# crowsonkb/k-diffusion

Hardware: NVIDIA H100
Metric: images/sec (256x256, Heun 50-step) (higher is better)
Workload: dtype bf16

## Files before the change

k-diffusion_b200/csrc/tc_attention.cu:

```cuda
#include "tc_common.cuh"
#include "tc_kernels.cuh"

namespace kdb {
namespace {

constexpr int ROWS = 128, DH = 64;
constexpr int TILE_BYTES = ROWS * DH * 2;
constexpr float LOG2E = 1.4426950408889634f;
constexpr int S_LD = ROWS + 4;

enum { MODE_WINDOW = 0, MODE_GLOBAL = 1, MODE_NA = 2 };

constexpr int NA_QH = 8, NA_QW = 16;
constexpr int NA_KH = 14, NA_KW = 22;
constexpr int NA_BLK_ROWS = 5;
constexpr int NA_BLK_KEYS = NA_BLK_ROWS * NA_KW;

struct AttnParams {
  bf16* out;
  const float* bound;
  int B, h, w, nh, shift, nblk;
};

struct Bars {
  uint64_t q, kv, kv_free;
};

template <int MODE, bool BOUNDED>
__global__ void __launch_bounds__(160, 1) attn_tc_kernel(const __grid_constant__ CUtensorMap tmap, const __grid_constant__ CUtensorMap tmap_kv,
                                                         const AttnParams p) {
  extern __shared__ uint8_t smem_raw[];
  uint8_t* base = reinterpret_cast<uint8_t*>((reinterpret_cast<uintptr_t>(smem_raw) + 1023) & ~(uintptr_t)1023);
  uint8_t* sQ = base;
  uint8_t* sK = base + TILE_BYTES;
  uint8_t* sV = base + 2 * TILE_BYTES;
  uint8_t* sP = (MODE == MODE_WINDOW) ? sQ : base + 3 * TILE_BYTES;
  float* sS = reinterpret_cast<float*>(base + (MODE == MODE_WINDOW ? 3 : 5) * TILE_BYTES);
  Bars* bars = reinterpret_cast<Bars*>(sS + ROWS * S_LD);

  const int warp = threadIdx.x >> 5, lane = threadIdx.x & 31;
  const int nh = p.nh;
  int b = blockIdx.z, head0, wi = 0, wj = 0, mtile = 0;
  if constexpr (MODE == MODE_WINDOW) {
    const int nww = p.w / 8;
    wi = blockIdx.x / nww;
    wj = blockIdx.x - wi * nww;
    head0 = blockIdx.y * 2;
  } else {
    mtile = blockIdx.x;
    head0 = blockIdx.y;
  }
  int qi0 = 0, qj0 = 0, r0 = 0, c0 = 0;
  if constexpr (MODE == MODE_NA) {
    const int nbw = p.w / NA_QW;
    qi0 = (blockIdx.x / nbw) * NA_QH;
    qj0 = (blockIdx.x % nbw) * NA_QW;
    r0 = min(max(qi0 - 3, 0), p.h - NA_KH);
    c0 = min(max(qj0 - 3, 0), p.w - NA_KW);
  }
  const int nblk = (MODE == MODE_WINDOW) ? 1 : p.nblk;
  constexpr bool bounded = BOUNDED;
  const bool two_pass = nblk > 1 && !bounded;
  const int n_iter = two_pass ? 2 * nblk : nblk;

  if (threadIdx.x == 0) {
    tc::tma_prefetch_desc(&tmap);
    tc::mbar_init(&bars->q, 1);
    tc::mbar_init(&bars->kv, 1);
    tc::mbar_init(&bars->kv_free, 4);
    tc::fence_barrier_init();
  }
  if constexpr (MODE == MODE_NA) {
    for (int i = threadIdx.x; i < (ROWS - NA_BLK_KEYS) * 8; i += blockDim.x)
      *reinterpret_cast<uint4*>(sV + NA_BLK_KEYS * 128 + i * 16) = make_uint4(0u, 0u, 0u, 0u);
    tc::fence_proxy_async();
  }
  __syncthreads();
  tc::pdl_wait();
  tc::pdl_launch_dependents();

  if (warp == 4) {
    if (tc::elect_one()) {
      auto load_window_tile = [&](uint8_t* dst, int t, uint64_t* bar) {
        if (p.shift == 0) {
#pragma unroll
          for (int hd = 0; hd < 2; ++hd) tc::tma_load_4d(dst + hd * 64 * 128, &tmap, bar, (t * nh + head0 + hd) * DH, wj * 8, wi * 8, b);
          return;
        }
#pragma unroll
        for (int hd = 0; hd < 2; ++hd)
#pragma unroll
          for (int quad = 0; quad < 4; ++quad) {
            const int r0 = (wi * 8 + (quad >> 1) * 4 - p.shift + p.h) % p.h;
            const int c0 = (wj * 8 + (quad & 1) * 4 - p.shift + p.w) % p.w;
            tc::tma_load_4d(dst + (hd * 64 + quad * 16) * 128, &tmap, bar, (t * nh + head0 + hd) * DH, c0, r0, b);
          }
      };
      tc::mbar_arrive_expect_tx(&bars->q, TILE_BYTES);
      if constexpr (MODE == MODE_WINDOW)
        load_window_tile(sQ, 0, &bars->q);
      else if constexpr (MODE == MODE_NA)
        tc::tma_load_4d(sQ, &tmap, &bars->q, head0 * DH, qj0, qi0, b);
      else
        tc::tma_load_3d(sQ, &tmap, &bars->q, head0 * DH, mtile * ROWS, b);
      for (int it = 0; it < n_iter; ++it) {
        const int j = it % nblk;
        const bool with_v = !two_pass || it >= nblk;
        if (it > 0) tc::mbar_wait(&bars->kv_free, (uint32_t)(it - 1) & 1u);
        constexpr uint32_t KV_BYTES = (MODE == MODE_NA) ? NA_BLK_KEYS * 128 : TILE_BYTES;
        tc::mbar_arrive_expect_tx(&bars->kv, with_v ? 2 * KV_BYTES : KV_BYTES);
        if constexpr (MODE == MODE_WINDOW) {
          load_window_tile(sK, 1, &bars->kv);
          load_window_tile(sV, 2, &bars->kv);
        } else if constexpr (MODE == MODE_NA) {
          tc::tma_load_4d(sK, &tmap_kv, &bars->kv, (nh + head0) * DH, c0, r0 + j * NA_BLK_ROWS, b);
          if (with_v) tc::tma_load_4d(sV, &tmap_kv, &bars->kv, (2 * nh + head0) * DH, c0, r0 + j * NA_BLK_ROWS, b);
        } else {
          tc::tma_load_3d(sK, &tmap, &bars->kv, (nh + head0) * DH, j * ROWS, b);
          if (with_v) tc::tma_load_3d(sV, &tmap, &bars->kv, (2 * nh + head0) * DH, j * ROWS, b);
        }
      }
    }
    return;
  }

  const int row = warp * 32 + lane;
  float m = -INFINITY, l = 0.f;
  const int hd = row >> 6, quad = (row & 63) >> 4;
  const bool seam_r = MODE == MODE_WINDOW && p.shift > 0 && wi == 0;
  const bool seam_c = MODE == MODE_WINDOW && p.shift > 0 && wj == 0;
  const int na_qi = qi0 + (row >> 4), na_qj = qj0 + (row & 15);
  const int na_rs = min(max(na_qi - 3, 0), p.h - 7), na_cs = min(max(na_qj - 3, 0), p.w - 7);
  auto key_ok = [&](int j, int t) -> bool {
    if constexpr (MODE != MODE_NA) return true;
    const int dr = (t * 745) >> 14;
    const int kr = r0 + j * NA_BLK_ROWS + dr, kc = c0 + (t - dr * NA_KW);
    return t < NA_BLK_KEYS && (unsigned)(kr - na_rs) < 7u && (unsigned)(kc - na_cs) < 7u;
  };
  const uint32_t q_addr = tc::smem_u32(sQ), k_addr = tc::smem_u32(sK), p_addr = tc::smem_u32(sP);
  const uint64_t vdesc = tc::smem_desc_mn_sw128(tc::smem_u32(sV), 1024, 1024);
  float o0[32], o1[32];
#pragma unroll
  for (int i = 0; i < 32; ++i) o0[i] = o1[i] = 0.f;
  tc::mbar_wait(&bars->q, 0);
  for (int it = 0; it < n_iter; ++it) {
    const int j = it % nblk;
    const int pass = (two_pass && it < nblk) ? 0 : 1;
    tc::mbar_wait(&bars->kv, (uint32_t)it & 1u);
#pragma unroll 1
    for (int h = 0; h < 2; ++h) {
      float s[64];
#pragma unroll
      for (int i = 0; i < 64; ++i) s[i] = 0.f;
      const uint64_t qd = tc::smem_desc_k_sw128(q_addr + (uint32_t)h * 8192u), kd = tc::smem_desc_k_sw128(k_addr);
      tc::wg_fence_acc(s);
      tc::wg_fence();
#pragma unroll
      for (int k = 0; k < DH / 16; ++k) tc::wgmma_128(s, qd + 2ull * k, kd + 2ull * k, 1u);
      tc::wg_commit();
      tc::wg_wait<0>();
      tc::wg_fence_acc(s);
      tc::acc_store(sS, S_LD, 64 * h, s);
    }
    tc::named_barrier_sync(1, 128);
    if (pass == 0) {
#pragma unroll 1
      for (int c = 0; c < 4; ++c) {
        float v[32];
        tc::acc_ld32(sS, S_LD, row, c * 32, v);
#pragma unroll
        for (int i = 0; i < 32; ++i) m = fmaxf(m, key_ok(j, c * 32 + i) ? v[i] : -INFINITY);
      }
    } else if constexpr (MODE != MODE_WINDOW) {
      if constexpr (bounded) m = __ldg(p.bound + head0);
      if (!two_pass && !bounded) {
        float mm = -INFINITY;
#pragma unroll 1
        for (int c2 = 0; c2 < 4; ++c2) {
          float u[32];
          tc::acc_ld32(sS, S_LD, row, c2 * 32, u);
#pragma unroll
          for (int i = 0; i < 32; ++i) mm = fmaxf(mm, u[i]);
        }
        m = mm;
      }
      const float mb = m * LOG2E;
#pragma unroll 1
      for (int c = 0; c < 4; ++c) {
        float v[32];
        tc::acc_ld32(sS, S_LD, row, c * 32, v);
        uint32_t pk[16];
#pragma unroll
        for (int i = 0; i < 16; ++i) {
          const float p0 = key_ok(j, c * 32 + 2 * i) ? exp2f(fmaf(v[2 * i], LOG2E, -mb)) : 0.f;
          const float p1 = key_ok(j, c * 32 + 2 * i + 1) ? exp2f(fmaf(v[2 * i + 1], LOG2E, -mb)) : 0.f;
          pk[i] = tc::pack_bf16x2(p0, p1);
          float q0, q1;
          tc::unpack_bf16x2(pk[i], q0, q1);
          l += q0 + q1;
        }
        uint8_t* pt = sP + (c >> 1) * TILE_BYTES;
#pragma unroll
        for (int jj = 0; jj < 4; ++jj)
          *reinterpret_cast<uint4*>(pt + tc::sw128_offset(row, (c & 1) * 4 + jj)) = make_uint4(pk[jj * 4], pk[jj * 4 + 1], pk[jj * 4 + 2], pk[jj * 4 + 3]);
      }
    } else {
      float v[64];
      {
        float t0[32], t1[32];
        tc::acc_ld32(sS, S_LD, row, hd * 64, t0);
        tc::acc_ld32(sS, S_LD, row, hd * 64 + 32, t1);
#pragma unroll
        for (int i = 0; i < 32; ++i) { v[i] = t0[i]; v[32 + i] = t1[i]; }
      }
      if constexpr (!bounded) {
#pragma unroll
        for (int i = 0; i < 64; ++i) {
          const int kq = i >> 4;
          const bool ok = (!seam_r || ((kq >> 1) == (quad >> 1))) && (!seam_c || ((kq & 1) == (quad & 1)));
          v[i] = ok ? v[i] : -INFINITY;
          m = fmaxf(m, v[i]);
        }
      } else {
        m = __ldg(p.bound + head0 + hd);
      }
      const float mb = m * LOG2E;
      uint8_t* own = sP + hd * TILE_BYTES;
      uint8_t* other = sP + (1 - hd) * TILE_BYTES;
#pragma unroll
      for (int jj = 0; jj < 8; ++jj) {
        uint32_t pk[4];
        bool ok = true;
        if constexpr (bounded) {
          const int kq = jj >> 1;
          ok = (!seam_r || ((kq >> 1) == (quad >> 1))) && (!seam_c || ((kq & 1) == (quad & 1)));
        }
#pragma unroll
        for (int t = 0; t < 4; ++t) {
          float p0 = exp2f(fmaf(v[jj * 8 + 2 * t], LOG2E, -mb)), p1 = exp2f(fmaf(v[jj * 8 + 2 * t + 1], LOG2E, -mb));
          if constexpr (bounded) {
            p0 = ok ? p0 : 0.f;
            p1 = ok ? p1 : 0.f;
          }
          pk[t] = tc::pack_bf16x2(p0, p1);
          float q0, q1;
          tc::unpack_bf16x2(pk[t], q0, q1);
          l += q0 + q1;
        }
        *reinterpret_cast<uint4*>(own + tc::sw128_offset(row, jj)) = make_uint4(pk[0], pk[1], pk[2], pk[3]);
        *reinterpret_cast<uint4*>(other + tc::sw128_offset(row, jj)) = make_uint4(0u, 0u, 0u, 0u);
      }
    }
    if (pass == 1) {
      tc::fence_proxy_async();
      tc::named_barrier_sync(1, 128);
      tc::wg_fence_acc(o0);
      tc::wg_fence_acc(o1);
      tc::wg_fence();
#pragma unroll
      for (int k = 0; k < ROWS / 16; ++k) {
        const uint32_t pa = p_addr + (uint32_t)((k >> 2) * TILE_BYTES);
        const uint64_t bd = vdesc + (uint64_t)(k * ((16 * 128) >> 4));
        tc::wgmma_64<1>(o0, tc::smem_desc_k_sw128(pa) + 2ull * (k & 3), bd, 1u);
        tc::wgmma_64<1>(o1, tc::smem_desc_k_sw128(pa + 8192u) + 2ull * (k & 3), bd, 1u);
      }
      tc::wg_commit();
      tc::wg_wait<0>();
      tc::wg_fence_acc(o0);
      tc::wg_fence_acc(o1);
    }
    tc::named_barrier_sync(1, 128);
    if (lane == 0 && it + 1 < n_iter) tc::mbar_arrive(&bars->kv_free);
  }
  tc::acc_store(sS, S_LD, 0, o0);
  tc::acc_store(sS, S_LD, 64, o1);
  tc::named_barrier_sync(1, 128);
  const float inv = 1.f / l;
  int64_t token;
  int head;
  if constexpr (MODE == MODE_WINDOW) {
    int oi, oj;
    if (p.shift == 0) {
      oi = wi * 8 + ((row & 63) >> 3);
      oj = wj * 8 + (row & 7);
    } else {
      const int lr = (row & 15) >> 2, lc = row & 3;
      oi = (wi * 8 + (quad >> 1) * 4 + lr - p.shift + p.h) % p.h;
      oj = (wj * 8 + (quad & 1) * 4 + lc - p.shift + p.w) % p.w;
    }
    token = (int64_t)oi * p.w + oj;
    head = head0 + hd;
  } else if constexpr (MODE == MODE_NA) {
    token = (int64_t)na_qi * p.w + na_qj;
    head = head0;
  } else {
    token = (int64_t)mtile * ROWS + row;
    head = head0;
  }
  uint4* dst = reinterpret_cast<uint4*>(p.out + (((int64_t)b * p.h * p.w + token) * nh + head) * DH);
#pragma unroll 1
  for (int c = 0; c < 2; ++c) {
// ... 106 lines not shown
```

k-diffusion_b200/csrc/tc_attn_block.cuh:

```cuda
#pragma once

constexpr int AB_C = 128;
constexpr int AB_XBUF = 2;
constexpr int AB_X_BYTES = 2 * A_STAGE_BYTES;
constexpr int AB_WQKV_KB = 3 * AB_C * 128;
constexpr int AB_WO_BYTES = 2 * A_STAGE_BYTES;
constexpr int AB_KV_BYTES = 64 * 128;
constexpr int AB_THREADS = 256 + 32;

struct AttnBlockBars {
  uint64_t w_full, x_full[AB_XBUF], x_empty[AB_XBUF];
};
constexpr size_t AB_SMEM = (size_t)AB_XBUF * AB_X_BYTES + 2 * AB_WQKV_KB + AB_WO_BYTES + 4 * AB_KV_BYTES + sizeof(AttnBlockBars) + 1024;

struct AttnBlockParams {
  const float* ss_in;
  float* ss_out;
  const float4* rope;
  const float* qk_scale;
  int h, w, shift, nwin;
};

__device__ __forceinline__ void ab_window(const AttnBlockParams& p, int win, int& b, int& wi, int& wj) {
  const int nww = p.w >> 3, per_img = (p.h >> 3) * nww;
  b = win / per_img;
  const int rem = win - b * per_img;
  wi = rem / nww;
  wj = rem - wi * nww;
}
__device__ __forceinline__ void ab_quad(const AttnBlockParams& p, int wi, int wj, int q, int& r, int& c) {
  r = (wi * 8 + (q >> 1) * 4 - p.shift + p.h) % p.h;
  c = (wj * 8 + (q & 1) * 4 - p.shift + p.w) % p.w;
}

__global__ void __launch_bounds__(AB_THREADS, 1) gemm_wg_attn_block_kernel(const __grid_constant__ CUtensorMap tmx,
                                                                          const __grid_constant__ CUtensorMap tmwq,
                                                                          const __grid_constant__ CUtensorMap tmwo, const AttnBlockParams p) {
  extern __shared__ uint8_t smem_raw[];
  uint8_t* base = reinterpret_cast<uint8_t*>((reinterpret_cast<uintptr_t>(smem_raw) + 1023) & ~(uintptr_t)1023);
  uint8_t* sX = base;
  uint8_t* sWQ = sX + AB_XBUF * AB_X_BYTES;
  uint8_t* sWO = sWQ + 2 * AB_WQKV_KB;
  uint8_t* sKV = sWO + AB_WO_BYTES;
  AttnBlockBars* bars = reinterpret_cast<AttnBlockBars*>(sKV + 4 * AB_KV_BYTES);
  const int pwarp = threadIdx.x >> 5, lane = threadIdx.x & 31;
  const int n_tiles = (p.nwin + 1) >> 1;
  const int n_local = (int)blockIdx.x < n_tiles ? (n_tiles - 1 - (int)blockIdx.x) / (int)gridDim.x + 1 : 0;

  if (threadIdx.x == 0) {
    tc::tma_prefetch_desc(&tmx);
    tc::tma_prefetch_desc(&tmwq);
    tc::tma_prefetch_desc(&tmwo);
    tc::mbar_init(&bars->w_full, 1);
    for (int i = 0; i < AB_XBUF; ++i) {
      tc::mbar_init(&bars->x_full[i], 1);
      tc::mbar_init(&bars->x_empty[i], 2);
    }
    tc::fence_barrier_init();
  }
  __syncthreads();
  tc::pdl_wait();
  tc::pdl_launch_dependents();

  if (pwarp == 8) {
    if (tc::elect_one()) {
      tc::mbar_arrive_expect_tx(&bars->w_full, 2 * AB_WQKV_KB + AB_WO_BYTES);
#pragma unroll
      for (int kb = 0; kb < 2; ++kb) {
        tc::tma_load_2d(sWQ + kb * AB_WQKV_KB, &tmwq, &bars->w_full, kb * BK, 0);
        tc::tma_load_2d(sWQ + kb * AB_WQKV_KB + 192 * 128, &tmwq, &bars->w_full, kb * BK, 192);
        tc::tma_load_2d(sWO + kb * A_STAGE_BYTES, &tmwo, &bars->w_full, kb * BK, 0);
      }
      for (int i = 0; i < n_local; ++i) {
        const int buf = i & 1;
        const int win0 = 2 * ((int)blockIdx.x + i * (int)gridDim.x);
        const int nw = p.nwin - win0 < 2 ? 1 : 2;
        tc::mbar_wait_nocall(&bars->x_empty[buf], (uint32_t)(((i >> 1) & 1) ^ 1));
        tc::mbar_arrive_expect_tx(&bars->x_full[buf], (uint32_t)nw * 2u * AB_KV_BYTES);
        for (int s = 0; s < nw; ++s) {
          int b, wi, wj;
          ab_window(p, win0 + s, b, wi, wj);
#pragma unroll
          for (int q = 0; q < 4; ++q) {
            int r, c;
            ab_quad(p, wi, wj, q, r, c);
#pragma unroll
            for (int kb = 0; kb < 2; ++kb)
              tc::tma_load_4d(sX + (size_t)buf * AB_X_BYTES + kb * A_STAGE_BYTES + s * AB_KV_BYTES + q * 2048, &tmx, &bars->x_full[buf], kb * BK, c, r, b);
          }
        }
      }
    }
    return;
  }

  const int wg = pwarp >> 2, t = threadIdx.x & 127;
  const int rw = 16 * (t >> 5) + (lane >> 2);
  const int r0 = 64 * wg + rw;
  const int cq = 2 * (lane & 3);
  const int quad = rw >> 4, lr = (rw & 15) >> 2, lc = rw & 3;
  uint8_t* sK = sKV + wg * 2 * AB_KV_BYTES;
  uint8_t* sV = sK + AB_KV_BYTES;
  const uint32_t wq_base = tc::smem_u32(sWQ), wo_base = tc::smem_u32(sWO);
  const uint64_t kdesc = tc::smem_desc_k_sw128(tc::smem_u32(sK));
  const uint64_t vdesc = tc::smem_desc_mn_sw128(tc::smem_u32(sV), 1024, 1024);
  const float sqs[2] = {sqrtf(__ldg(p.qk_scale)), sqrtf(__ldg(p.qk_scale + 1))};
  const int T = p.h * p.w;
  constexpr float LOG2E = 1.4426950408889634f;

  auto store_tile = [&](uint8_t* dst, const float (&a)[32]) {
#pragma unroll
    for (int j = 0; j < 8; ++j) {
      *reinterpret_cast<uint32_t*>(dst + tc::sw128_offset(rw, j) + cq * 2) = tc::pack_bf16x2(a[4 * j], a[4 * j + 1]);
      *reinterpret_cast<uint32_t*>(dst + tc::sw128_offset(rw + 8, j) + cq * 2) = tc::pack_bf16x2(a[4 * j + 2], a[4 * j + 3]);
    }
  };
  auto qk_norm_rope = [&](float (&a)[32], int hd, int tok0, int tok1) {
    float4 cs[2][2];
#pragma unroll
    for (int jj = 0; jj < 2; ++jj) {
      const float4* tb = p.rope + (int64_t)(hd * 8 + 4 * jj + (lane & 3)) * T;
      cs[0][jj] = __ldg(tb + tok0);
      cs[1][jj] = __ldg(tb + tok1);
    }
    const float sq = sqs[hd];
    float s0 = 0.f, s1 = 0.f;
#pragma unroll
    for (int j = 0; j < 8; ++j) {
      s0 = fmaf(a[4 * j], a[4 * j], fmaf(a[4 * j + 1], a[4 * j + 1], s0));
      s1 = fmaf(a[4 * j + 2], a[4 * j + 2], fmaf(a[4 * j + 3], a[4 * j + 3], s1));
    }
    s0 += __shfl_xor_sync(0xffffffffu, s0, 1);
    s0 += __shfl_xor_sync(0xffffffffu, s0, 2);
    s1 += __shfl_xor_sync(0xffffffffu, s1, 1);
    s1 += __shfl_xor_sync(0xffffffffu, s1, 2);
    const float sc[2] = {sq * rsqrtf(s0 + 1e-6f), sq * rsqrtf(s1 + 1e-6f)};
#pragma unroll
    for (int jj = 0; jj < 2; ++jj)
#pragma unroll
      for (int rr = 0; rr < 2; ++rr) {
        const int i1 = 4 * jj + 2 * rr, i2 = 4 * (jj + 2) + 2 * rr;
        const float4 c = cs[rr][jj];
        const float x1a = a[i1], x1b = a[i1 + 1], x2a = a[i2], x2b = a[i2 + 1];
        a[i1] = fmaf(x2a, -c.z, x1a * c.x) * sc[rr];
        a[i1 + 1] = fmaf(x2b, -c.w, x1b * c.y) * sc[rr];
        a[i2] = fmaf(x1a, c.z, x2a * c.x) * sc[rr];
        a[i2 + 1] = fmaf(x1b, c.w, x2b * c.y) * sc[rr];
      }
#pragma unroll
    for (int j = 4; j < 8; ++j) {
      a[4 * j] *= sc[0];
      a[4 * j + 1] *= sc[0];
      a[4 * j + 2] *= sc[1];
      a[4 * j + 3] *= sc[1];
    }
  };
  auto to_afrag = [](const float (&a)[32], uint32_t (&f)[16]) {
#pragma unroll
    for (int i = 0; i < 16; ++i) f[i] = tc::pack_bf16x2(a[2 * i], a[2 * i + 1]);
  };

  tc::mbar_wait_nocall(&bars->w_full, 0);
  for (int i = 0; i < n_local; ++i) {
    const int buf = i & 1;
    const int win = 2 * ((int)blockIdx.x + i * (int)gridDim.x) + wg;
    if (win >= p.nwin) continue;
    int b, wi, wj, qr, qc;
    ab_window(p, win, b, wi, wj);
    ab_quad(p, wi, wj, quad, qr, qc);
    const int tok0 = (qr + lr) * p.w + qc + lc, tok1 = tok0 + 2 * p.w;
    const int64_t m0 = (int64_t)b * T + tok0, m1 = (int64_t)b * T + tok1;
    const float rstd0 = rsqrtf(__ldg(p.ss_in + m0 * SS_PARTS) / (float)AB_C + 1e-6f);
    const float rstd1 = rsqrtf(__ldg(p.ss_in + m1 * SS_PARTS) / (float)AB_C + 1e-6f);
    const bool seam_r = p.shift > 0 && wi == 0, seam_c = p.shift > 0 && wj == 0;
    tc::mbar_wait_nocall(&bars->x_full[buf], (uint32_t)((i >> 1) & 1));
    const uint32_t xa = tc::smem_u32(sX + (size_t)buf * AB_X_BYTES) + (uint32_t)wg * AB_KV_BYTES;
    uint32_t of[2][16];
#pragma unroll 1
    for (int hd = 0; hd < 2; ++hd) {
      float va[32], ka[32], qa[32];
#pragma unroll
      for (int j = 0; j < 32; ++j) va[j] = ka[j] = qa[j] = 0.f;
      tc::wg_fence_acc(va);
      tc::wg_fence_acc(ka);
      tc::wg_fence();
      auto project = [&](float (&d)[32], int third) {
#pragma unroll
        for (int kb = 0; kb < 2; ++kb) {
          const uint64_t ad = tc::smem_desc_k_sw128(xa + (uint32_t)(kb * A_STAGE_BYTES));
          const uint64_t bd = tc::smem_desc_k_sw128(wq_base + (uint32_t)(kb * AB_WQKV_KB + (third * AB_C + 64 * hd) * 128));
#pragma unroll
          for (int k = 0; k < 4; ++k) tc::wgmma_64<0>(d, ad + 2ull * k, bd + 2ull * k, 1u);
        }
        tc::wg_commit();
      };
      project(va, 2);
      project(ka, 1);
      if (hd == 1) tc::named_barrier_sync(1 + wg, 128);
      tc::wg_wait<1>();
      tc::wg_fence_acc(va);
#pragma unroll
      for (int j = 0; j < 8; ++j) {
        va[4 * j] *= rstd0;
        va[4 * j + 1] *= rstd0;
        va[4 * j + 2] *= rstd1;
        va[4 * j + 3] *= rstd1;
      }
      store_tile(sV, va);
      tc::wg_fence_acc(qa);
      tc::wg_fence();
      project(qa, 0);
      tc::wg_wait<1>();
      tc::wg_fence_acc(ka);
      qk_norm_rope(ka, hd, tok0, tok1);
      store_tile(sK, ka);
      tc::wg_wait<0>();
      tc::wg_fence_acc(qa);
      qk_norm_rope(qa, hd, tok0, tok1);
      uint32_t qf[16];
      to_afrag(qa, qf);
      tc::fence_proxy_async();
      tc::named_barrier_sync(1 + wg, 128);
      float s[32];
#pragma unroll
      for (int j = 0; j < 32; ++j) s[j] = 0.f;
      tc::wg_fence_acc(s);
      tc::wg_fence_acc(qf);
      tc::wg_fence();
#pragma unroll
      for (int kk = 0; kk < 4; ++kk) {
        const uint32_t a[4] = {qf[4 * kk], qf[4 * kk + 1], qf[4 * kk + 2], qf[4 * kk + 3]};
        tc::wgmma_64_rs<0>(s, a, kdesc + 2ull * kk, 1u);
      }
      tc::wg_commit();
      tc::wg_wait<0>();
      tc::wg_fence_acc(s);
      float mx0 = -INFINITY, mx1 = -INFINITY;
#pragma unroll
      for (int j = 0; j < 8; ++j) {
        const int kq = j >> 1;
        const bool ok = (!seam_r || ((kq >> 1) == (quad >> 1))) && (!seam_c || ((kq & 1) == (quad & 1)));
        if (!ok) s[4 * j] = s[4 * j + 1] = s[4 * j + 2] = s[4 * j + 3] = -INFINITY;
        mx0 = fmaxf(mx0, fmaxf(s[4 * j], s[4 * j + 1]));
        mx1 = fmaxf(mx1, fmaxf(s[4 * j + 2], s[4 * j + 3]));
      }
      mx0 = fmaxf(mx0, __shfl_xor_sync(0xffffffffu, mx0, 1));
      mx0 = fmaxf(mx0, __shfl_xor_sync(0xffffffffu, mx0, 2));
      mx1 = fmaxf(mx1, __shfl_xor_sync(0xffffffffu, mx1, 1));
      mx1 = fmaxf(mx1, __shfl_xor_sync(0xffffffffu, mx1, 2));
      const float mb0 = mx0 * LOG2E, mb1 = mx1 * LOG2E;
      uint32_t pf[16];
      float l0 = 0.f, l1 = 0.f;
#pragma unroll
      for (int i2 = 0; i2 < 16; ++i2) {
        const float mb = (i2 & 1) ? mb1 : mb0;
        pf[i2] = tc::pack_bf16x2(exp2f(fmaf(s[2 * i2], LOG2E, -mb)), exp2f(fmaf(s[2 * i2 + 1], LOG2E, -mb)));
        float e0, e1;
        tc::unpack_bf16x2(pf[i2], e0, e1);
        if (i2 & 1) l1 += e0 + e1;
        else l0 += e0 + e1;
      }
      l0 += __shfl_xor_sync(0xffffffffu, l0, 1);
      l0 += __shfl_xor_sync(0xffffffffu, l0, 2);
      l1 += __shfl_xor_sync(0xffffffffu, l1, 1);
      l1 += __shfl_xor_sync(0xffffffffu, l1, 2);
      float o[32];
#pragma unroll
      for (int j = 0; j < 32; ++j) o[j] = 0.f;
      tc::wg_fence_acc(o);
      tc::wg_fence_acc(pf);
      tc::wg_fence();
#pragma unroll
      for (int kk = 0; kk < 4; ++kk) {
        const uint32_t a[4] = {pf[4 * kk], pf[4 * kk + 1], pf[4 * kk + 2], pf[4 * kk + 3]};
        tc::wgmma_64_rs<1>(o, a, vdesc + (uint64_t)(kk * ((16 * 128) >> 4)), 1u);
      }
      tc::wg_commit();
      tc::wg_wait<0>();
      tc::wg_fence_acc(o);
      const float inv0 = __frcp_rn(l0), inv1 = __frcp_rn(l1);
#pragma unroll
      for (int j = 0; j < 8; ++j) {
        o[4 * j] *= inv0;
        o[4 * j + 1] *= inv0;
        o[4 * j + 2] *= inv1;
        o[4 * j + 3] *= inv1;
      }
      uint32_t oh[16];
      to_afrag(o, oh);
#pragma unroll
      for (int j = 0; j < 16; ++j) {
        of[0][j] = hd == 0 ? oh[j] : of[0][j];
        of[1][j] = hd == 0 ? of[1][j] : oh[j];
      }
    }
    float acc[64];
#pragma unroll
    for (int j = 0; j < 64; ++j) acc[j] = 0.f;
    tc::wg_fence_acc(acc);
    tc::wg_fence_acc(of[0]);
    tc::wg_fence_acc(of[1]);
    tc::wg_fence();
#pragma unroll
    for (int hd = 0; hd < 2; ++hd) {
      const uint64_t od = tc::smem_desc_k_sw128(wo_base + (uint32_t)(hd * A_STAGE_BYTES));
#pragma unroll
      for (int kk = 0; kk < 4; ++kk) {
        const uint32_t a[4] = {of[hd][4 * kk], of[hd][4 * kk + 1], of[hd][4 * kk + 2], of[hd][4 * kk + 3]};
        tc::wgmma_128_rs(acc, a, od + 2ull * kk, 1u);
      }
    }
    tc::wg_commit();
    tc::wg_wait<0>();
    tc::wg_fence_acc(acc);
    uint8_t* xt = sX + (size_t)buf * AB_X_BYTES;
    float ss0 = 0.f, ss1 = 0.f;
#pragma unroll
    for (int j = 0; j < 16; ++j) {
      uint8_t* sub = xt + (j >> 3) * A_STAGE_BYTES;
      uint32_t* p0 = reinterpret_cast<uint32_t*>(sub + tc::sw128_offset(r0, j & 7) + cq * 2);
      uint32_t* p1 = reinterpret_cast<uint32_t*>(sub + tc::sw128_offset(r0 + 8, j & 7) + cq * 2);
      const uint32_t x0 = *p0, x1 = *p1;
      const float a0 = acc[4 * j] + __uint_as_float(x0 << 16), a1 = acc[4 * j + 1] + __uint_as_float(x0 & 0xffff0000u);
      const float b0 = acc[4 * j + 2] + __uint_as_float(x1 << 16), b1 = acc[4 * j + 3] + __uint_as_float(x1 & 0xffff0000u);
      ss0 = fmaf(a0, a0, fmaf(a1, a1, ss0));
      ss1 = fmaf(b0, b0, fmaf(b1, b1, ss1));
      *p0 = tc::pack_bf16x2(a0, a1);
      *p1 = tc::pack_bf16x2(b0, b1);
    }
    ss0 += __shfl_xor_sync(0xffffffffu, ss0, 1);
    ss0 += __shfl_xor_sync(0xffffffffu, ss0, 2);
    ss1 += __shfl_xor_sync(0xffffffffu, ss1, 1);
    ss1 += __shfl_xor_sync(0xffffffffu, ss1, 2);
    if ((lane & 3) == 0) {
      p.ss_out[m0 * SS_PARTS] = ss0;
      p.ss_out[m1 * SS_PARTS] = ss1;
    }
    tc::fence_proxy_async();
    tc::named_barrier_sync(1 + wg, 128);
    if (t == 0) {
#pragma unroll
      for (int q = 0; q < 4; ++q) {
        int r, c;
        ab_quad(p, wi, wj, q, r, c);
#pragma unroll
        for (int kb = 0; kb < 2; ++kb) tc::tma_store_4d(&tmx, xt + kb * A_STAGE_BYTES + wg * AB_KV_BYTES + q * 2048, kb * BK, c, r, b);
      }
      tc::tma_store_commit();
      tc::tma_store_wait_read();
      tc::mbar_arrive(&bars->x_empty[buf]);
    }
  }
}

inline bool attn_block_supported(int h, int w, int C, int nh, int e, int attn_type, int attn_param, int shift) {
  return C == AB_C && nh == 2 && e == 64 && attn_type == KDB_ATTN_SHIFTED_WINDOW && attn_param == 8 && (shift == 0 || shift == 4) && h > 0 &&
         w > 0 && h % 8 == 0 && w % 8 == 0;
}

int launch_attn_block_impl(bf16* x, const bf16* w_qkv, const bf16* w_out, const float2* rope, const float* qk_scale, int B, int h, int w,
                           int shift, const float* ss_in, float* ss_out, cudaStream_t st) {
  CUtensorMap tx, twq, two;
  int rc;
  const uint64_t dims[4] = {(uint64_t)AB_C, (uint64_t)w, (uint64_t)h, (uint64_t)B};
  const uint64_t strides[3] = {(uint64_t)AB_C * 2, (uint64_t)AB_C * 2 * w, (uint64_t)AB_C * 2 * w * h};
  const uint32_t box[4] = {BK, 4, 4, 1};
  if ((rc = make_tmap_bf16(&tx, x, 4, dims, strides, box))) return rc;
  if ((rc = tmap_2d(&twq, w_qkv, AB_C, 3 * AB_C, BK, 192))) return rc;
  if ((rc = tmap_2d(&two, w_out, AB_C, AB_C, BK, AB_C))) return rc;
  static bool attr_set = false;
  if (!attr_set) {
// ... 11 lines not shown
```

k-diffusion_b200/csrc/tc_ffn_fused.cuh:

```cuda
#pragma once

constexpr int FF_C = 128;
constexpr int FF_CH = 64;
constexpr int FF_XBUF = 2, FF_WU = 3, FF_WD = 3;
constexpr int FF_X_BYTES = 2 * A_STAGE_BYTES;
constexpr int FF_WU_BYTES = 2 * A_STAGE_BYTES;
constexpr int FF_WD_BYTES = A_STAGE_BYTES;
constexpr int FF_THREADS = 256 + 32;

struct FfnBars {
  uint64_t x_full[FF_XBUF], x_empty[FF_XBUF];
  uint64_t wu_full[FF_WU], wu_empty[FF_WU];
  uint64_t wd_full[FF_WD], wd_empty[FF_WD];
};
constexpr size_t FF_SMEM = (size_t)FF_XBUF * FF_X_BYTES + (size_t)FF_WU * FF_WU_BYTES + (size_t)FF_WD * FF_WD_BYTES + sizeof(FfnBars) + 1024;

struct FfnParams {
  const float* ss_in;
  float* ss_out;
  int64_t M;
  int nc;
};

__global__ void __launch_bounds__(FF_THREADS, 1) ffn_fused_kernel(const __grid_constant__ CUtensorMap tmx, const __grid_constant__ CUtensorMap tmwu,
                                                                 const __grid_constant__ CUtensorMap tmwd, const __grid_constant__ CUtensorMap tmo,
                                                                 const FfnParams p) {
  extern __shared__ uint8_t smem_raw[];
  uint8_t* base = reinterpret_cast<uint8_t*>((reinterpret_cast<uintptr_t>(smem_raw) + 1023) & ~(uintptr_t)1023);
  uint8_t* sX = base;
  uint8_t* sWU = sX + FF_XBUF * FF_X_BYTES;
  uint8_t* sWD = sWU + FF_WU * FF_WU_BYTES;
  FfnBars* bars = reinterpret_cast<FfnBars*>(sWD + FF_WD * FF_WD_BYTES);
  const int pwarp = threadIdx.x >> 5, lane = threadIdx.x & 31;
  const int nc = p.nc;
  const int m_tiles = (int)(p.M / BM);
  const int n_local = (int)blockIdx.x < m_tiles ? (m_tiles - 1 - (int)blockIdx.x) / (int)gridDim.x + 1 : 0;

  if (threadIdx.x == 0) {
    tc::tma_prefetch_desc(&tmx);
    tc::tma_prefetch_desc(&tmwu);
    tc::tma_prefetch_desc(&tmwd);
    tc::tma_prefetch_desc(&tmo);
    for (int i = 0; i < FF_XBUF; ++i) {
      tc::mbar_init(&bars->x_full[i], 1);
      tc::mbar_init(&bars->x_empty[i], 2);
    }
    for (int i = 0; i < FF_WU; ++i) {
      tc::mbar_init(&bars->wu_full[i], 1);
      tc::mbar_init(&bars->wu_empty[i], 8);
    }
    for (int i = 0; i < FF_WD; ++i) {
      tc::mbar_init(&bars->wd_full[i], 1);
      tc::mbar_init(&bars->wd_empty[i], 8);
    }
    tc::fence_barrier_init();
  }
  __syncthreads();
  tc::pdl_wait();
  tc::pdl_launch_dependents();

  if (pwarp == 8) {
    if (tc::elect_one()) {
      uint32_t su = 0, pu = 0, sd = 0, pd = 0;
      for (int i = 0; i < n_local; ++i) {
        const int buf = i & 1;
        tc::mbar_wait(&bars->x_empty[buf], (uint32_t)(((i >> 1) & 1) ^ 1));
        tc::mbar_arrive_expect_tx(&bars->x_full[buf], FF_X_BYTES);
        const int m0 = ((int)blockIdx.x + i * (int)gridDim.x) * BM;
        tc::tma_load_2d(sX + (size_t)buf * FF_X_BYTES, &tmx, &bars->x_full[buf], 0, m0);
        tc::tma_load_2d(sX + (size_t)buf * FF_X_BYTES + A_STAGE_BYTES, &tmx, &bars->x_full[buf], BK, m0);
        for (int c = 0; c < nc; ++c) {
          tc::mbar_wait(&bars->wu_empty[su], pu ^ 1u);
          tc::mbar_arrive_expect_tx(&bars->wu_full[su], FF_WU_BYTES);
          tc::tma_load_2d(sWU + (size_t)su * FF_WU_BYTES, &tmwu, &bars->wu_full[su], 0, c * 128);
          tc::tma_load_2d(sWU + (size_t)su * FF_WU_BYTES + A_STAGE_BYTES, &tmwu, &bars->wu_full[su], BK, c * 128);
          if (++su == FF_WU) {
            su = 0;
            pu ^= 1u;
          }
          tc::mbar_wait(&bars->wd_empty[sd], pd ^ 1u);
          tc::mbar_arrive_expect_tx(&bars->wd_full[sd], FF_WD_BYTES);
          tc::tma_load_2d(sWD + (size_t)sd * FF_WD_BYTES, &tmwd, &bars->wd_full[sd], c * FF_CH, 0);
          if (++sd == FF_WD) {
            sd = 0;
            pd ^= 1u;
          }
        }
      }
    }
    return;
  }

  const int wg = pwarp >> 2, t = threadIdx.x & 127;
  const int r0 = 64 * wg + 16 * (t >> 5) + (lane >> 2);
  const int cq = 2 * (lane & 3);
  const uint32_t wu_base = tc::smem_u32(sWU), wd_base = tc::smem_u32(sWD);
  uint32_t su = 0, pu = 0, sd = 0, pd = 0;
  for (int i = 0; i < n_local; ++i) {
    const int buf = i & 1;
    const int64_t m0 = ((int64_t)blockIdx.x + (int64_t)i * gridDim.x) * BM;
    const float rstd0 = rsqrtf(__ldg(p.ss_in + (m0 + r0) * SS_PARTS) / (float)FF_C + 1e-6f);
    const float rstd1 = rsqrtf(__ldg(p.ss_in + (m0 + r0 + 8) * SS_PARTS) / (float)FF_C + 1e-6f);
    const tc::f32x2 g0 = tc::pk2(rstd0, rstd0), g1 = tc::pk2(rstd1, rstd1), h0 = tc::pk2(0.5f * rstd0, 0.5f * rstd0), h1 = tc::pk2(0.5f * rstd1, 0.5f * rstd1);
    tc::mbar_wait(&bars->x_full[buf], (uint32_t)((i >> 1) & 1));
    const uint32_t xa = tc::smem_u32(sX + (size_t)buf * FF_X_BYTES) + (uint32_t)wg * 8192u;
    float acc2[64];
#pragma unroll
    for (int j = 0; j < 64; ++j) acc2[j] = 0.f;
    for (int c = 0; c < nc; ++c) {
      float acc1[64];
#pragma unroll
      for (int j = 0; j < 64; ++j) acc1[j] = 0.f;
      tc::mbar_wait(&bars->wu_full[su], pu);
      const uint32_t wa = wu_base + su * (uint32_t)FF_WU_BYTES;
      tc::wg_fence_acc(acc1);
      tc::wg_fence();
#pragma unroll
      for (int kb = 0; kb < 2; ++kb) {
        const uint64_t ad = tc::smem_desc_k_sw128(xa + (uint32_t)(kb * A_STAGE_BYTES)), bd = tc::smem_desc_k_sw128(wa + (uint32_t)(kb * A_STAGE_BYTES));
#pragma unroll
        for (int k = 0; k < 4; ++k) tc::wgmma_128(acc1, ad + 2ull * k, bd + 2ull * k, 1u);
      }
      tc::wg_commit();
      tc::wg_wait<0>();
      tc::wg_fence_acc(acc1);
      if (lane == 0) tc::mbar_arrive(&bars->wu_empty[su]);
      if (++su == FF_WU) {
        su = 0;
        pu ^= 1u;
      }
      uint32_t hreg[16];
#pragma unroll
      for (int q = 0; q < 8; ++q) {
        const tc::f32x2 v0 = tc::mul2(tc::pk2(acc1[8 * q], acc1[8 * q + 1]), h0), v1 = tc::mul2(tc::pk2(acc1[8 * q + 2], acc1[8 * q + 3]), h1);
        const tc::f32x2 q0 = tc::mul2(tc::pk2(acc1[8 * q + 4], acc1[8 * q + 5]), g0), q1 = tc::mul2(tc::pk2(acc1[8 * q + 6], acc1[8 * q + 7]), g1);
        float o0, o1, o2, o3;
        tc::upk2(tc::geglu2(v0, q0), o0, o1);
        tc::upk2(tc::geglu2(v1, q1), o2, o3);
        hreg[(q >> 1) * 4 + (q & 1) * 2 + 0] = tc::pack_bf16x2(o0, o1);
        hreg[(q >> 1) * 4 + (q & 1) * 2 + 1] = tc::pack_bf16x2(o2, o3);
      }
      tc::mbar_wait(&bars->wd_full[sd], pd);
      const uint64_t bd = tc::smem_desc_k_sw128(wd_base + sd * (uint32_t)FF_WD_BYTES);
      tc::wg_fence_acc(acc2);
      tc::wg_fence_acc(hreg);
      tc::wg_fence();
#pragma unroll
      for (int kk = 0; kk < 4; ++kk) {
        const uint32_t a[4] = {hreg[4 * kk], hreg[4 * kk + 1], hreg[4 * kk + 2], hreg[4 * kk + 3]};
        tc::wgmma_128_rs(acc2, a, bd + 2ull * kk, 1u);
      }
      tc::wg_commit();
      tc::wg_wait<0>();
      tc::wg_fence_acc(acc2);
      if (lane == 0) tc::mbar_arrive(&bars->wd_empty[sd]);
      if (++sd == FF_WD) {
        sd = 0;
        pd ^= 1u;
      }
    }
    uint8_t* xt = sX + (size_t)buf * FF_X_BYTES;
    float ss0 = 0.f, ss1 = 0.f;
#pragma unroll
    for (int j = 0; j < 16; ++j) {
      uint8_t* sub = xt + (j >> 3) * SUB_TILE_BYTES;
      const uint32_t in16 = (uint32_t)(cq * 2);
      uint32_t* p0 = reinterpret_cast<uint32_t*>(sub + tc::sw128_offset(r0, j & 7) + in16);
      uint32_t* p1 = reinterpret_cast<uint32_t*>(sub + tc::sw128_offset(r0 + 8, j & 7) + in16);
      const uint32_t x0 = *p0, x1 = *p1;
      const float a0 = acc2[4 * j] + __uint_as_float(x0 << 16), a1 = acc2[4 * j + 1] + __uint_as_float(x0 & 0xffff0000u);
      const float b0 = acc2[4 * j + 2] + __uint_as_float(x1 << 16), b1 = acc2[4 * j + 3] + __uint_as_float(x1 & 0xffff0000u);
      ss0 = fmaf(a0, a0, fmaf(a1, a1, ss0));
      ss1 = fmaf(b0, b0, fmaf(b1, b1, ss1));
      *p0 = tc::pack_bf16x2(a0, a1);
      *p1 = tc::pack_bf16x2(b0, b1);
    }
    ss0 += __shfl_xor_sync(0xffffffffu, ss0, 1);
    ss0 += __shfl_xor_sync(0xffffffffu, ss0, 2);
    ss1 += __shfl_xor_sync(0xffffffffu, ss1, 1);
    ss1 += __shfl_xor_sync(0xffffffffu, ss1, 2);
    if (p.ss_out != nullptr && (lane & 3) == 0) {
      p.ss_out[(m0 + r0) * SS_PARTS] = ss0;
      p.ss_out[(m0 + r0 + 8) * SS_PARTS] = ss1;
    }
    tc::fence_proxy_async();
    tc::named_barrier_sync(1 + wg, 128);
    if (t == 0) {
      tc::tma_store_2d(&tmo, xt + wg * 8192, 0, (int)m0 + 64 * wg);
      tc::tma_store_2d(&tmo, xt + SUB_TILE_BYTES + wg * 8192, 64, (int)m0 + 64 * wg);
      tc::tma_store_commit();
      tc::tma_store_wait_read();
      tc::mbar_arrive(&bars->x_empty[buf]);
    }
  }
}

inline bool ffn_fused_supported(int64_t M, int C, int dff) { return C == FF_C && M > 0 && M % BM == 0 && dff % FF_CH == 0 && dff / FF_CH >= 3; }

int launch_ffn_fused_impl(bf16* x, const bf16* w_up_il, const bf16* w_down, int64_t M, int dff, const float* ss_in, float* ss_out, cudaStream_t st) {
  CUtensorMap tx, twu, twd, to;
  int rc;
  if ((rc = tmap_2d(&tx, x, FF_C, (uint64_t)M, BK, BM))) return rc;
  if ((rc = tmap_2d(&twu, w_up_il, FF_C, (uint64_t)2 * dff, BK, 128))) return rc;
  if ((rc = tmap_2d(&twd, w_down, (uint64_t)dff, FF_C, BK, FF_C))) return rc;
  if ((rc = tmap_2d(&to, x, FF_C, (uint64_t)M, 64, BM / 2))) return rc;
  static bool attr_set = false;
  if (!attr_set) {
    KDB_CUDA(cudaFuncSetAttribute(ffn_fused_kernel, cudaFuncAttributeMaxDynamicSharedMemorySize, (int)FF_SMEM));
    attr_set = true;
  }
  FfnParams p{ss_in, ss_out, M, dff / FF_CH};
  const int64_t m_tiles = M / BM;
  KDB_CUDA(launch_pdl(ffn_fused_kernel, dim3((unsigned)(m_tiles < num_sms() ? m_tiles : num_sms())), dim3(FF_THREADS), FF_SMEM, st, tx, twu,
                      twd, to, p));
  KDB_LAUNCH_CHECK(F_GEMM_TC, st);
  return 0;
}
```

Before: 112.2.

## Software-pipeline fused FFN GEMMs with ping-pong warpgroups and register reallocation

The fused FFN consumer loop is restructured so each chunk's up-projection wgmma is issued while the previous chunk's GEGLU and down-projection run. Named barriers make the two consumer warpgroups alternate issue (ping-pong), so one group's tensor-core work hides the other's elementwise math. The producer is widened to a full warpgroup that gives up registers via setmaxnreg_dec, letting consumers grow to 232 registers. The attention block now issues all three QKV projections before waiting and loads the rope tables once, and mbarrier waits switch to a non-call variant. The risks are added barrier coupling between warpgroups and register-pressure changes.

```diff
diff --git a/k-diffusion_b200/csrc/tc_attention.cu b/k-diffusion_b200/csrc/tc_attention.cu
--- a/k-diffusion_b200/csrc/tc_attention.cu
+++ b/k-diffusion_b200/csrc/tc_attention.cu
@@ -106,7 +106,7 @@
       for (int it = 0; it < n_iter; ++it) {
         const int j = it % nblk;
         const bool with_v = !two_pass || it >= nblk;
-        if (it > 0) tc::mbar_wait(&bars->kv_free, (uint32_t)(it - 1) & 1u);
+        if (it > 0) tc::mbar_wait_nocall(&bars->kv_free, (uint32_t)(it - 1) & 1u);
         constexpr uint32_t KV_BYTES = (MODE == MODE_NA) ? NA_BLK_KEYS * 128 : TILE_BYTES;
         tc::mbar_arrive_expect_tx(&bars->kv, with_v ? 2 * KV_BYTES : KV_BYTES);
         if constexpr (MODE == MODE_WINDOW) {
@@ -142,11 +142,11 @@
   float o0[32], o1[32];
 #pragma unroll
   for (int i = 0; i < 32; ++i) o0[i] = o1[i] = 0.f;
-  tc::mbar_wait(&bars->q, 0);
+  tc::mbar_wait_nocall(&bars->q, 0);
   for (int it = 0; it < n_iter; ++it) {
     const int j = it % nblk;
     const int pass = (two_pass && it < nblk) ? 0 : 1;
-    tc::mbar_wait(&bars->kv, (uint32_t)it & 1u);
+    tc::mbar_wait_nocall(&bars->kv, (uint32_t)it & 1u);
 #pragma unroll 1
     for (int h = 0; h < 2; ++h) {
       float s[64];
diff --git a/k-diffusion_b200/csrc/tc_attn_block.cuh b/k-diffusion_b200/csrc/tc_attn_block.cuh
--- a/k-diffusion_b200/csrc/tc_attn_block.cuh
+++ b/k-diffusion_b200/csrc/tc_attn_block.cuh
@@ -6,7 +6,7 @@
 constexpr int AB_WQKV_KB = 3 * AB_C * 128;
 constexpr int AB_WO_BYTES = 2 * A_STAGE_BYTES;
 constexpr int AB_KV_BYTES = 64 * 128;
-constexpr int AB_THREADS = 256 + 32;
+constexpr int AB_THREADS = 256 + 128;
 
 struct AttnBlockBars {
   uint64_t w_full, x_full[AB_XBUF], x_empty[AB_XBUF];
@@ -62,8 +62,9 @@
   tc::pdl_wait();
   tc::pdl_launch_dependents();
 
-  if (pwarp == 8) {
-    if (tc::elect_one()) {
+  if (pwarp >= 8) {
+    tc::setmaxnreg_dec<40>();
+    if (pwarp == 8 && tc::elect_one()) {
       tc::mbar_arrive_expect_tx(&bars->w_full, 2 * AB_WQKV_KB + AB_WO_BYTES);
 #pragma unroll
       for (int kb = 0; kb < 2; ++kb) {
@@ -94,6 +95,7 @@
     return;
   }
 
+  tc::setmaxnreg_inc<232>();
   const int wg = pwarp >> 2, t = threadIdx.x & 127;
   const int rw = 16 * (t >> 5) + (lane >> 2);
   const int r0 = 64 * wg + rw;
@@ -115,14 +117,7 @@
       *reinterpret_cast<uint32_t*>(dst + tc::sw128_offset(rw + 8, j) + cq * 2) = tc::pack_bf16x2(a[4 * j + 2], a[4 * j + 3]);
     }
   };
-  auto qk_norm_rope = [&](float (&a)[32], int hd, int tok0, int tok1) {
-    float4 cs[2][2];
-#pragma unroll
-    for (int jj = 0; jj < 2; ++jj) {
-      const float4* tb = p.rope + (int64_t)(hd * 8 + 4 * jj + (lane & 3)) * T;
-      cs[0][jj] = __ldg(tb + tok0);
-      cs[1][jj] = __ldg(tb + tok1);
-    }
+  auto qk_norm_rope = [&](float (&a)[32], int hd, const float4 (&cs)[2][2]) {
     const float sq = sqs[hd];
     float s0 = 0.f, s1 = 0.f;
 #pragma unroll
@@ -183,6 +178,7 @@
       for (int j = 0; j < 32; ++j) va[j] = ka[j] = qa[j] = 0.f;
       tc::wg_fence_acc(va);
       tc::wg_fence_acc(ka);
+      tc::wg_fence_acc(qa);
       tc::wg_fence();
       auto project = [&](float (&d)[32], int third) {
 #pragma unroll
@@ -196,8 +192,16 @@
       };
       project(va, 2);
       project(ka, 1);
+      project(qa, 0);
+      float4 cs[2][2];
+#pragma unroll
+      for (int jj = 0; jj < 2; ++jj) {
+        const float4* tb = p.rope + (int64_t)(hd * 8 + 4 * jj + (lane & 3)) * T;
+        cs[0][jj] = __ldg(tb + tok0);
+        cs[1][jj] = __ldg(tb + tok1);
+      }
       if (hd == 1) tc::named_barrier_sync(1 + wg, 128);
-      tc::wg_wait<1>();
+      tc::wg_wait<2>();
       tc::wg_fence_acc(va);
 #pragma unroll
       for (int j = 0; j < 8; ++j) {
@@ -207,16 +211,13 @@
         va[4 * j + 3] *= rstd1;
       }
       store_tile(sV, va);
-      tc::wg_fence_acc(qa);
-      tc::wg_fence();
-      project(qa, 0);
       tc::wg_wait<1>();
       tc::wg_fence_acc(ka);
-      qk_norm_rope(ka, hd, tok0, tok1);
+      qk_norm_rope(ka, hd, cs);
       store_tile(sK, ka);
       tc::wg_wait<0>();
       tc::wg_fence_acc(qa);
-      qk_norm_rope(qa, hd, tok0, tok1);
+      qk_norm_rope(qa, hd, cs);
       uint32_t qf[16];
       to_afrag(qa, qf);
       tc::fence_proxy_async();
diff --git a/k-diffusion_b200/csrc/tc_ffn_fused.cuh b/k-diffusion_b200/csrc/tc_ffn_fused.cuh
--- a/k-diffusion_b200/csrc/tc_ffn_fused.cuh
+++ b/k-diffusion_b200/csrc/tc_ffn_fused.cuh
@@ -6,7 +6,7 @@
 constexpr int FF_X_BYTES = 2 * A_STAGE_BYTES;
 constexpr int FF_WU_BYTES = 2 * A_STAGE_BYTES;
 constexpr int FF_WD_BYTES = A_STAGE_BYTES;
-constexpr int FF_THREADS = 256 + 32;
+constexpr int FF_THREADS = 256 + 128;
 
 struct FfnBars {
   uint64_t x_full[FF_XBUF], x_empty[FF_XBUF];
@@ -59,18 +59,19 @@
   tc::pdl_wait();
   tc::pdl_launch_dependents();
 
-  if (pwarp == 8) {
-    if (tc::elect_one()) {
+  if (pwarp >= 8) {
+    tc::setmaxnreg_dec<40>();
+    if (pwarp == 8 && tc::elect_one()) {
       uint32_t su = 0, pu = 0, sd = 0, pd = 0;
       for (int i = 0; i < n_local; ++i) {
         const int buf = i & 1;
-        tc::mbar_wait(&bars->x_empty[buf], (uint32_t)(((i >> 1) & 1) ^ 1));
+        tc::mbar_wait_nocall(&bars->x_empty[buf], (uint32_t)(((i >> 1) & 1) ^ 1));
         tc::mbar_arrive_expect_tx(&bars->x_full[buf], FF_X_BYTES);
         const int m0 = ((int)blockIdx.x + i * (int)gridDim.x) * BM;
         tc::tma_load_2d(sX + (size_t)buf * FF_X_BYTES, &tmx, &bars->x_full[buf], 0, m0);
         tc::tma_load_2d(sX + (size_t)buf * FF_X_BYTES + A_STAGE_BYTES, &tmx, &bars->x_full[buf], BK, m0);
         for (int c = 0; c < nc; ++c) {
-          tc::mbar_wait(&bars->wu_empty[su], pu ^ 1u);
+          tc::mbar_wait_nocall(&bars->wu_empty[su], pu ^ 1u);
           tc::mbar_arrive_expect_tx(&bars->wu_full[su], FF_WU_BYTES);
           tc::tma_load_2d(sWU + (size_t)su * FF_WU_BYTES, &tmwu, &bars->wu_full[su], 0, c * 128);
           tc::tma_load_2d(sWU + (size_t)su * FF_WU_BYTES + A_STAGE_BYTES, &tmwu, &bars->wu_full[su], BK, c * 128);
@@ -78,7 +79,7 @@
             su = 0;
             pu ^= 1u;
           }
-          tc::mbar_wait(&bars->wd_empty[sd], pd ^ 1u);
+          tc::mbar_wait_nocall(&bars->wd_empty[sd], pd ^ 1u);
           tc::mbar_arrive_expect_tx(&bars->wd_full[sd], FF_WD_BYTES);
           tc::tma_load_2d(sWD + (size_t)sd * FF_WD_BYTES, &tmwd, &bars->wd_full[sd], c * FF_CH, 0);
           if (++sd == FF_WD) {
@@ -91,73 +92,96 @@
     return;
   }
 
+  tc::setmaxnreg_inc<232>();
   const int wg = pwarp >> 2, t = threadIdx.x & 127;
   const int r0 = 64 * wg + 16 * (t >> 5) + (lane >> 2);
   const int cq = 2 * (lane & 3);
   const uint32_t wu_base = tc::smem_u32(sWU), wd_base = tc::smem_u32(sWD);
   uint32_t su = 0, pu = 0, sd = 0, pd = 0;
+  bool first_block = true;
+  float acc1[64], acc2[64];
+  uint32_t hreg[16];
   for (int i = 0; i < n_local; ++i) {
     const int buf = i & 1;
     const int64_t m0 = ((int64_t)blockIdx.x + (int64_t)i * gridDim.x) * BM;
     const float rstd0 = rsqrtf(__ldg(p.ss_in + (m0 + r0) * SS_PARTS) / (float)FF_C + 1e-6f);
     const float rstd1 = rsqrtf(__ldg(p.ss_in + (m0 + r0 + 8) * SS_PARTS) / (float)FF_C + 1e-6f);
     const tc::f32x2 g0 = tc::pk2(rstd0, rstd0), g1 = tc::pk2(rstd1, rstd1), h0 = tc::pk2(0.5f * rstd0, 0.5f * rstd0), h1 = tc::pk2(0.5f * rstd1, 0.5f * rstd1);
-    tc::mbar_wait(&bars->x_full[buf], (uint32_t)((i >> 1) & 1));
+    tc::mbar_wait_nocall(&bars->x_full[buf], (uint32_t)((i >> 1) & 1));
     const uint32_t xa = tc::smem_u32(sX + (size_t)buf * FF_X_BYTES) + (uint32_t)wg * 8192u;
-    float acc2[64];
 #pragma unroll
     for (int j = 0; j < 64; ++j) acc2[j] = 0.f;
-    for (int c = 0; c < nc; ++c) {
-      float acc1[64];
+    for (int c = 0; c <= nc; ++c) {
+      if (c > 0) {
+        tc::wg_wait<0>();
+        tc::wg_fence_acc(acc1);
+        tc::wg_fence_acc(acc2);
+        tc::wg_fence_acc(hreg);
+        if (lane == 0) tc::mbar_arrive(&bars->wu_empty[su]);
+        if (++su == FF_WU) {
+          su = 0;
+          pu ^= 1u;
+        }
+        if (c > 1) {
+          if (lane == 0) tc::mbar_arrive(&bars->wd_empty[sd]);
+          if (++sd == FF_WD) {
+            sd = 0;
+            pd ^= 1u;
+          }
+        }
+#pragma unroll
+        for (int q = 0; q < 8; ++q) {
+          const tc::f32x2 v0 = tc::mul2(tc::pk2(acc1[8 * q], acc1[8 * q + 1]), h0), v1 = tc::mul2(tc::pk2(acc1[8 * q + 2], acc1[8 * q + 3]), h1);
+          const tc::f32x2 q0 = tc::mul2(tc::pk2(acc1[8 * q + 4], acc1[8 * q + 5]), g0), q1 = tc::mul2(tc::pk2(acc1[8 * q + 6], acc1[8 * q + 7]), g1);
+          float o0, o1, o2, o3;
+          tc::upk2(tc::geglu2(v0, q0), o0, o1);
+          tc::upk2(tc::geglu2(v1, q1), o2, o3);
+          hreg[(q >> 1) * 4 + (q & 1) * 2 + 0] = tc::pack_bf16x2(o0, o1);
+          hreg[(q >> 1) * 4 + (q & 1) * 2 + 1] = tc::pack_bf16x2(o2, o3);
+        }
+      }
 #pragma unroll
       for (int j = 0; j < 64; ++j) acc1[j] = 0.f;
-      tc::mbar_wait(&bars->wu_full[su], pu);
-      const uint32_t wa = wu_base + su * (uint32_t)FF_WU_BYTES;
       tc::wg_fence_acc(acc1);
-      tc::wg_fence();
-#pragma unroll
-      for (int kb = 0; kb < 2; ++kb) {
-        const uint64_t ad = tc::smem_desc_k_sw128(xa + (uint32_t)(kb * A_STAGE_BYTES)), bd = tc::smem_desc_k_sw128(wa + (uint32_t)(kb * A_STAGE_BYTES));
-#pragma unroll
-        for (int k = 0; k < 4; ++k) tc::wgmma_128(acc1, ad + 2ull * k, bd + 2ull * k, 1u);
-      }
-      tc::wg_commit();
-      tc::wg_wait<0>();
-      tc::wg_fence_acc(acc1);
-      if (lane == 0) tc::mbar_arrive(&bars->wu_empty[su]);
-      if (++su == FF_WU) {
-        su = 0;
-        pu ^= 1u;
-      }
-      uint32_t hreg[16];
-#pragma unroll
-      for (int q = 0; q < 8; ++q) {
-        const tc::f32x2 v0 = tc::mul2(tc::pk2(acc1[8 * q], acc1[8 * q + 1]), h0), v1 = tc::mul2(tc::pk2(acc1[8 * q + 2], acc1[8 * q + 3]), h1);
-        const tc::f32x2 q0 = tc::mul2(tc::pk2(acc1[8 * q + 4], acc1[8 * q + 5]), g0), q1 = tc::mul2(tc::pk2(acc1[8 * q + 6], acc1[8 * q + 7]), g1);
-        float o0, o1, o2, o3;
-        tc::upk2(tc::geglu2(v0, q0), o0, o1);
-        tc::upk2(tc::geglu2(v1, q1), o2, o3);
-        hreg[(q >> 1) * 4 + (q & 1) * 2 + 0] = tc::pack_bf16x2(o0, o1);
-        hreg[(q >> 1) * 4 + (q & 1) * 2 + 1] = tc::pack_bf16x2(o2, o3);
-      }
-      tc::mbar_wait(&bars->wd_full[sd], pd);
-      const uint64_t bd = tc::smem_desc_k_sw128(wd_base + sd * (uint32_t)FF_WD_BYTES);
-      tc::wg_fence_acc(acc2);
-      tc::wg_fence_acc(hreg);
-      tc::wg_fence();
-#pragma unroll
-      for (int kk = 0; kk < 4; ++kk) {
-        const uint32_t a[4] = {hreg[4 * kk], hreg[4 * kk + 1], hreg[4 * kk + 2], hreg[4 * kk + 3]};
-        tc::wgmma_128_rs(acc2, a, bd + 2ull * kk, 1u);
-      }
-      tc::wg_commit();
-      tc::wg_wait<0>();
-      tc::wg_fence_acc(acc2);
-      if (lane == 0) tc::mbar_arrive(&bars->wd_empty[sd]);
-      if (++sd == FF_WD) {
-        sd = 0;
-        pd ^= 1u;
-      }
+      if (wg == 1) tc::named_barrier_sync(4, 256);
+      else if (!first_block) tc::named_barrier_sync(3, 256);
+      first_block = false;
+      if (c > 0) {
+        tc::mbar_wait_nocall(&bars->wd_full[sd], pd);
+        const uint64_t bd = tc::smem_desc_k_sw128(wd_base + sd * (uint32_t)FF_WD_BYTES);
+        tc::wg_fence_acc(acc2);
+        tc::wg_fence_acc(hreg);
+        tc::wg_fence();
+#pragma unroll
+        for (int kk = 0; kk < 4; ++kk) {
+          const uint32_t a[4] = {hreg[4 * kk], hreg[4 * kk + 1], hreg[4 * kk + 2], hreg[4 * kk + 3]};
+          tc::wgmma_128_rs(acc2, a, bd + 2ull * kk, 1u);
+        }
+        tc::wg_commit();
+      }
+      if (c < nc) {
+        tc::mbar_wait_nocall(&bars->wu_full[su], pu);
+        const uint32_t wa = wu_base + su * (uint32_t)FF_WU_BYTES;
+        tc::wg_fence_acc(acc1);
+        tc::wg_fence();
+#pragma unroll
+        for (int kb = 0; kb < 2; ++kb) {
+          const uint64_t ad = tc::smem_desc_k_sw128(xa + (uint32_t)(kb * A_STAGE_BYTES)), bd = tc::smem_desc_k_sw128(wa + (uint32_t)(kb * A_STAGE_BYTES));
+#pragma unroll
+          for (int k = 0; k < 4; ++k) tc::wgmma_128(acc1, ad + 2ull * k, bd + 2ull * k, 1u);
+        }
+        tc::wg_commit();
+      }
+      if (wg == 0) tc::named_barrier_arrive(4, 256);
+      else if (c < nc || i + 1 < n_local) tc::named_barrier_arrive(3, 256);
+    }
+    tc::wg_wait<0>();
+    tc::wg_fence_acc(acc2);
+    tc::wg_fence_acc(hreg);
+    if (lane == 0) tc::mbar_arrive(&bars->wd_empty[sd]);
+    if (++sd == FF_WD) {
+      sd = 0;
+      pd ^= 1u;
     }
     uint8_t* xt = sX + (size_t)buf * FF_X_BYTES;
     float ss0 = 0.f, ss1 = 0.f;
```

New measurement: 118.7, median of 6. +5.8%, better.
